# EPOCHDevs/PandasArrow

Measured on AMD Instinct MI355X. Metric: Grows/sec hash group-by-sum, 1e9 int64 rows x 1e6 keys, higher is better.
Workload: dtype f64; 1 GPU; group_by(int64 key).agg(sum,mean,count), 1e+09 rows / 1e+06 keys, 1 GPU; rows=1000000000, keys=1000000, rows_per_gpu=1000000000, parity=bit-exact vs Arrow-order pairwise sum

## Files before the change

### pandasarrow_amd/csrc/compact.hpp

```cpp
#pragma once
#include "pdx_common.hpp"
#include "scan.hpp"

namespace pdx {

constexpr int kCompactBlock = 256;
constexpr int kCompactItems = 16;
constexpr int kCompactTile = kCompactBlock * kCompactItems;

template <typename Pred>
__global__ void __launch_bounds__(kCompactBlock) k_compact_count(int64_t n, Pred pred, int64_t* __restrict__ block_counts) {
  __shared__ int wave_tot[4];
  const int lane = threadIdx.x & 63, wave = threadIdx.x >> 6;
  int64_t base = (int64_t)blockIdx.x * kCompactTile + wave * (64 * kCompactItems);
  int cnt = 0;
  for (int s = 0; s < kCompactItems; ++s) {
    int64_t i = base + s * 64 + lane;
    bool p = i < n && pred(i);
    cnt += __popcll(__ballot(p));
  }
  if (lane == 0) wave_tot[wave] = cnt;
  __syncthreads();
  if (threadIdx.x == 0) block_counts[blockIdx.x] = (int64_t)wave_tot[0] + wave_tot[1] + wave_tot[2] + wave_tot[3];
}
// ... 11 lines not shown
  }
  if (lane == 0) wave_tot[wave] = cnt;
  __syncthreads();
  int64_t pos = block_offsets[blockIdx.x];
  for (int w = 0; w < wave; ++w) pos += wave_tot[w];
  const uint64_t lt = (1ull << lane) - 1ull;
  for (int s = 0; s < kCompactItems; ++s) {
    int64_t i = base + s * 64 + lane;
    bool p = i < n && pred(i);
    uint64_t b = __ballot(p);
    if (p) emit(pos + __popcll(b & lt), i);
    pos += __popcll(b);
  }
}

template <typename Pred, typename Emit>
int compact_indices(int64_t n, Pred pred, Emit emit, int64_t* total_host , Scratch& s,
                    hipStream_t st) {
  if (total_host) *total_host = 0;
  if (n <= 0) return PDX_OK;
  int64_t nblocks = ceil_div(n, kCompactTile);
  int64_t* counts = s.get<int64_t>((size_t)nblocks);
  int64_t* total = s.get<int64_t>(1);
  PDX_SCRATCH_CHECK(s);
  hipLaunchKernelGGL((k_compact_count<Pred>), dim3((unsigned)nblocks), dim3(kCompactBlock), 0, st, n, pred, counts);
  PDX_TRY((device_exclusive_scan<int64_t, SumOp>(counts, counts, nblocks, total, s, st)));
  hipLaunchKernelGGL((k_compact_write<Pred, Emit>), dim3((unsigned)nblocks), dim3(kCompactBlock), 0, st, n, pred, emit, counts);
  PDX_LAUNCH_CHECK();
  if (!total_host) return PDX_OK;
  PDX_HIP(hipMemcpyAsync(total_host, total, sizeof(int64_t), hipMemcpyDeviceToHost, st));
  PDX_HIP(hipStreamSynchronize(st));
  return PDX_OK;
}

template <typename Pred>
int count_if(int64_t n, Pred pred, int64_t* total_host, Scratch& s, hipStream_t st) {
  *total_host = 0;
  if (n <= 0) return PDX_OK;
  int64_t nblocks = ceil_div(n, kCompactTile);
  int64_t* counts = s.get<int64_t>((size_t)nblocks);
  int64_t* total = s.get<int64_t>(1);
  PDX_SCRATCH_CHECK(s);
  hipLaunchKernelGGL((k_compact_count<Pred>), dim3((unsigned)nblocks), dim3(kCompactBlock), 0, st, n, pred, counts);
// ... 21 lines not shown
```

### pandasarrow_amd/csrc/gb_create.hpp

```cpp
#pragma once

struct CreateTuning {
  bool sorted = true;
  bool dense = true;
  bool dense_lds = true;
  bool dense_speculate = true;
  int speculate_bits = 20;
  int64_t prefix_per_slot = 0;
  int partition = 1;
  bool hash_rows = false;
  bool hash_lds = true;
  int64_t head_rows = 0;
  bool hash_split = true;
  bool hash_debug = false;
  static CreateTuning read() {
    CreateTuning t;
    auto off = [](const char* name) { const char* e = getenv(name); return e && e[0] == '0'; };
    t.sorted = !off("PDX_GROUPBY_SORTED");
    t.dense = !off("PDX_GROUPBY_DENSE");
    t.dense_lds = !off("PDX_DENSE_LDS");
    t.dense_speculate = !off("PDX_DENSE_SPECULATE");
    if (const char* e = getenv("PDX_DENSE_SPECULATE_BITS")) t.speculate_bits = atoi(e);
    if (const char* e = getenv("PDX_DENSE_PREFIX_PER_SLOT")) if (atoi(e) > 0) t.prefix_per_slot = atoi(e);
    if (const char* e = getenv("PDX_HASH_PARTITION")) t.partition = e[0] == '0' ? 0 : e[0] == '2' ? 2 : 1;
// ... 12 lines not shown
  const uint8_t* valid;
  int64_t key_off;
  int64_t n;
  Scratch& s;
  hipStream_t st;
  const CreateTuning& t;
  HashCtl* ctl;
};

struct SlotDomain {
  Slot* table = nullptr;
  unsigned int* dense_first = nullptr;
  long long dense_min = 0;
  unsigned int dense_mask = 0, null_slot = 0, region = 0;
  int64_t nslots = 0;
};

struct PoolFree {
  void operator()(void* p) const { pool_free(p); }
};
using TableBlock = std::unique_ptr<Slot, PoolFree>;
static Slot* alloc_table(unsigned int cap) { return static_cast<Slot*>(pool_alloc(((size_t)cap + 2) * sizeof(Slot))); }

constexpr KeyRange kNoKeys{0x7FFFFFFFFFFFFFFFll, (long long)0x8000000000000000ull, 0, 0};
static void widen_range(KeyRange& r, const KeyRange& w) {
  if (!w.any) return;
  r.vmin = std::min(r.vmin, w.vmin);
  r.vmax = std::max(r.vmax, w.vmax);
  r.any = 1;
}

struct KeySample {
  bool maybe_sorted = false;
  KeyRange range = kNoKeys;
};
static int sample_keys(const CreateCtx& c, bool want_sorted, bool want_range, KeySample* out) {
  if (!want_sorted && !want_range) return PDX_OK;
  KeyRange hsv[64];
  unsigned int hflags[4] = {0, 0, 0, 4u};
  unsigned int* flags = c.s.get<unsigned int>(4);
  KeyRange* dsample = c.s.get<KeyRange>(64);
  if (c.s.failed) return PDX_OOM;
  if (want_sorted) {
    PDX_HIP(hipMemsetAsync(flags, 0, 4 * sizeof(unsigned int), c.st));
    hipLaunchKernelGGL(k_sample_descents, dim3(64), dim3(1024), 0, c.st, c.keys, c.valid, c.key_off, c.n, flags + 3);
    PDX_HIP(hipMemcpyAsync(hflags, flags, sizeof(hflags), hipMemcpyDeviceToHost, c.st));
  }
  if (want_range) {
    hipLaunchKernelGGL(k_sample_key_range, dim3(64), dim3(1024), 0, c.st, c.keys, c.valid, c.key_off, c.n, dsample);
    PDX_HIP(hipMemcpyAsync(hsv, dsample, sizeof(hsv), hipMemcpyDeviceToHost, c.st));
  }
  PDX_LAUNCH_CHECK();
  PDX_HIP(hipStreamSynchronize(c.st));
  out->maybe_sorted = want_sorted && !(hflags[3] & 4u) && (hflags[3] & 3u) != 3u;
  if (want_range)
    for (const KeyRange& w : hsv) widen_range(out->range, w);
  return PDX_OK;
}

static int64_t dense_prefix_rows(const CreateCtx& c, int64_t nslots) {
  int64_t per_slot = c.t.prefix_per_slot;
  if (per_slot <= 0) per_slot = c.n < ((int64_t)1 << 29) ? 8 : ((nslots + 31) >> 5) <= kDenseLdsWords ? 4 : 16;
  const int64_t prefix = std::min<int64_t>(c.n, std::max<int64_t>((int64_t)1 << 22, per_slot * nslots));
  return std::min<int64_t>(c.n, round_up(prefix, kSortTile));
}

static int build_dense_domain(const CreateCtx& c, long long mn, unsigned int mask, unsigned int null_slot, int64_t nslots, KeyRange* range_out,
                              unsigned int** first_out) {
  pdx_groupby* gb = c.gb;
  hipStream_t st = c.st;
  const int64_t n = c.n;
  unsigned int* dense_first = *first_out = c.s.get<unsigned int>((size_t)nslots);
  if (c.s.failed) return PDX_OOM;
  hipMemsetAsync(dense_first, 0xFF, (size_t)nslots * sizeof(unsigned int), st);
  const int64_t ntiles = ceil_div(n, kSortTile), nchunks = ceil_div(ntiles, kColChunk);
  const int bits0 = make_sort_plan(ilog2((uint64_t)nslots), sort_max_bits()).bits[0];
  const int64_t prefix = dense_prefix_rows(c, nslots);
  const bool fuse = bits0 >= 4 && bits0 <= 8;
  const int64_t nwords = (nslots + 31) >> 5;
  const int64_t tile_first_tail = prefix / kSortTile;
  const bool lds_bitmap = fuse && c.t.dense_lds && prefix < n && nwords <= kDenseLdsWords && ntiles - tile_first_tail >= 256;
  if (range_out && !(fuse && prefix < n)) return fail(PDX_DEVICE, "dense_build: fused key range needs the histogram tail");
  uint32_t* chunk_sum = nullptr;
  if (fuse) {
    gb->pass0_off = gb->own<uint32_t>((size_t)ntiles << bits0);
    chunk_sum = c.s.get<uint32_t>((size_t)(nchunks + 1) << bits0);
    if (!gb->pass0_off || c.s.failed) return PDX_OOM;
  }
  KeyRange* wg_range = nullptr;
  long long *tile_min = nullptr, *tile_max = nullptr;
  if (range_out) {
    wg_range = c.s.get<KeyRange>((size_t)kCUs);
    if (c.s.failed) return PDX_OOM;
    if (!lds_bitmap) {
      tile_min = c.s.get<long long>((size_t)ntiles);
      tile_max = c.s.get<long long>((size_t)ntiles);
      if (c.s.failed) return PDX_OOM;
    }
  }
  {
    PDX_PROFILE("dense_slots", st);
    if (prefix < n && fuse && (lds_bitmap || range_out))
      hipLaunchKernelGGL(k_dense_slots<false>, dim3(grid_for(prefix, 256, 8)), dim3(256), 0, st, c.keys, c.valid, c.key_off, prefix, mn, mask, null_slot,
                         dense_first, gb->slot_of_row);
    else
      hipLaunchKernelGGL(k_dense_slots<true>, dim3(grid_for(prefix, 256, 8)), dim3(256), 0, st, c.keys, c.valid, c.key_off, prefix, mn, mask, null_slot,
                         dense_first, gb->slot_of_row);
    if (prefix < n) {
// ... 14 lines not shown
                               mask, null_slot, seen, prefix, dense_first, gb->slot_of_row, gb->pass0_off, tile_min, tile_max);
          else
            hipLaunchKernelGGL((k_dense_slots_tail_hist<b()>), dim3(tail_tiles), dim3(kSortBlock), 0, st, c.keys, c.valid, c.key_off, tile_first_tail, n, mn,
                               mask, null_slot, seen, prefix, dense_first, gb->slot_of_row, gb->pass0_off, (long long*)nullptr, (long long*)nullptr);
        });
    }
  }
  PDX_LAUNCH_CHECK();
  if (fuse) {
    if (!lds_bitmap && !range_out)
      with_digit_bits<4, 8>(bits0, [&](auto b) {
        hipLaunchKernelGGL((k_radix_hist<b()>), dim3((unsigned)ceil_div(prefix, kSortTile)), dim3(kSortBlock), 0, st, gb->slot_of_row, prefix, 0, gb->pass0_off);
      });
    PDX_TRY(radix_scan_dispatch(bits0, gb->pass0_off, ntiles, chunk_sum, true, st));
  }
  if (range_out && !lds_bitmap) {
    long long lo = 0, hi = 0, dummy = 0;
    PDX_TRY(minmax_i64_host(tile_min, ntiles, &lo, &dummy, c.s, st));
    PDX_TRY(minmax_i64_host(tile_max, ntiles, &dummy, &hi, c.s, st));
    *range_out = KeyRange{lo, hi, lo <= hi ? 1 : 0, 0};
  } else if (range_out) {
    std::vector<KeyRange> h((size_t)kCUs);
    PDX_HIP(hipMemcpyAsync(h.data(), wg_range, sizeof(KeyRange) * kCUs, hipMemcpyDeviceToHost, st));
    PDX_HIP(hipStreamSynchronize(st));
    *range_out = kNoKeys;
    for (const KeyRange& w : h) widen_range(*range_out, w);
  }
  return PDX_OK;
}

struct KeyRangeFacts {
  MinMaxPartial<long long> mm;
  bool have_mm = false;
  bool not_dense = false;
};

static unsigned long long dense_limit(int64_t n) { return std::min<unsigned long long>(1ull << 26, (unsigned long long)n * 4 + 1024); }

static int try_dense_speculative(const CreateCtx& c, const KeyRange& hs, SlotDomain* d, KeyRangeFacts* f) {
  pdx_groupby* gb = c.gb;
  const int64_t n = c.n;
  const unsigned long long dense_lim = dense_limit(n);
  int b = 64;
  if (hs.any) {
    const unsigned long long span_s = (unsigned long long)hs.vmax - (unsigned long long)hs.vmin;
    b = 4;
    while (b < 64 && (span_s >> b)) ++b;
    if (span_s >= dense_lim) f->not_dense = true;
  }
  if (!(b <= c.t.speculate_bits && b <= 26 && (1ull << b) <= dense_lim && (int64_t)16 * (((int64_t)1 << b) + 1) + 2 * kSortTile < n)) return PDX_OK;
  const unsigned int mask = (1u << b) - 1, null_slot = 1u << b;
  const int64_t nslots = (int64_t)null_slot + (c.valid ? 1 : 0);
  const size_t mark = gb->owned.size();
  gb->slot_of_row = gb->own<uint32_t>((size_t)n);
  if (!gb->slot_of_row) return PDX_OOM;
  KeyRange exact;
  unsigned int* first = nullptr;
  PDX_TRY(build_dense_domain(c, 0, mask, null_slot, nslots, &exact, &first));
  f->mm.vmin = exact.vmin;
  f->mm.vmax = exact.vmax;
  f->mm.rmin = f->mm.rmax = exact.any ? 0 : -1;
  f->have_mm = true;
  if (exact.any && (unsigned long long)exact.vmax - (unsigned long long)exact.vmin <= mask) {
    gb->dense = 1;
    d->dense_first = first;
    d->dense_min = exact.vmin;
    d->dense_mask = mask;
    d->null_slot = null_slot;
    d->nslots = nslots;
    return PDX_OK;
  }
  while (gb->owned.size() > mark) {
    pool_free(gb->owned.back());
    gb->owned.pop_back();
  }
  gb->slot_of_row = nullptr;
  gb->pass0_off = nullptr;
  return PDX_OK;
}

static int try_dense_exact(const CreateCtx& c, SlotDomain* d, KeyRangeFacts* f) {
  pdx_groupby* gb = c.gb;
  if (!f->have_mm) {
    PDX_TRY(minmax_keys_host(c.keys, c.valid, c.key_off, c.n, &f->mm, c.s, c.st));
    f->have_mm = true;
  }
  if (f->mm.rmin >= 0) {
    const unsigned long long span = (unsigned long long)f->mm.vmax - (unsigned long long)f->mm.vmin;
    if (span >= dense_limit(c.n)) return PDX_OK;
    d->dense_min = f->mm.vmin;
    d->null_slot = (unsigned int)span + 1;
    d->nslots = (int64_t)d->null_slot + 1;
  } else {
    d->null_slot = 0;
    d->nslots = 1;
  }
  gb->dense = 1;
  gb->slot_of_row = gb->own<uint32_t>((size_t)c.n);
  if (!gb->slot_of_row) return PDX_OOM;
  return build_dense_domain(c, d->dense_min, 0, d->null_slot, d->nslots, nullptr, &d->dense_first);
}

struct HashPartition {
  int64_t ntiles = 0, nchunks = 0;
  long long* keys_part = nullptr;
  unsigned int pb = kPartBits;
  uint32_t* bucket_starts = nullptr;
  bool idx16_written = false;
  bool lds_failed_at_pb = false;
};

static int partition_by_bucket(const CreateCtx& c, HashPartition* hp) {
  pdx_groupby* gb = c.gb;
  hipStream_t st = c.st;
  const int64_t n = c.n;
// ... 220 lines not shown
  gb->owned.push_back(table.get());
  d->table = table.release();
  d->null_slot = cap;
  d->nslots = (int64_t)cap + 2;
  return PDX_OK;
}

static int finish_group_ids(const CreateCtx& c, const SlotDomain& d) {
  pdx_groupby* gb = c.gb;
  Scratch& s = c.s;
  hipStream_t st = c.st;
  const int64_t n = c.n, nslots = d.nslots;
  gb->nslots = nslots;
  gb->slot_bits = ilog2((uint64_t)nslots);
  gb->gid_of_slot = gb->own<uint32_t>((size_t)nslots);
  uint32_t* occ_slot_tmp = s.get<uint32_t>((size_t)std::min<int64_t>(nslots, n + 2));
  uint32_t* occ_first_tmp = s.get<uint32_t>((size_t)std::min<int64_t>(nslots, n + 2));
  if (s.failed || !gb->gid_of_slot) return PDX_OOM;
  int64_t G = 0;
  PDX_TRY(compact_indices(nslots, OccPred{d.table, d.dense_first, d.region, d.null_slot},
                          OccEmit{d.table, d.dense_first, d.region, d.null_slot, occ_slot_tmp, occ_first_tmp}, &G, s, st));
  gb->G = G;
  gb->occ_slot = gb->own<uint32_t>((size_t)G);
  gb->gid_of_occ = gb->own<uint32_t>((size_t)G);
  gb->uniques = gb->own<int64_t>((size_t)G);
  gb->unique_ok = gb->own<uint8_t>((size_t)G);
  gb->first_rows = gb->own<int64_t>((size_t)G);
  if (s.failed || !gb->occ_slot || !gb->gid_of_occ || !gb->uniques || !gb->unique_ok || !gb->first_rows) return PDX_OOM;
  hipMemcpyAsync(gb->occ_slot, occ_slot_tmp, (size_t)G * sizeof(uint32_t), hipMemcpyDeviceToDevice, st);
  const bool rank_by_sort = G > ((int64_t)1 << 22) && G * 8 > n;
  const int g = grid_for(G, 256);
  if (rank_by_sort) {
    uint32_t* k0 = s.get<uint32_t>((size_t)G);
    uint32_t* v0 = s.get<uint32_t>((size_t)G);
    uint32_t* k1 = s.get<uint32_t>((size_t)G);
    uint32_t* v1 = s.get<uint32_t>((size_t)G);
    PDX_SCRATCH_CHECK(s);
    const uint32_t *ks = nullptr, *vs = nullptr;
    PDX_TRY(radix_sort_pairs<uint32_t>(occ_first_tmp, occ_slot_tmp, k0, v0, k1, v1, G, ilog2((uint64_t)n + 1) < 31 ? ilog2((uint64_t)n + 1) : 31, &ks, &vs, true,
                                       s, st));
    hipLaunchKernelGGL(k_assign_gids, dim3(g), dim3(256), 0, st, d.table, d.dense_min, d.dense_mask, gb->gid_of_slot, ks, vs, G, d.null_slot, gb->uniques,
                       gb->unique_ok, gb->first_rows, d.region);
    hipLaunchKernelGGL(k_gid_of_occ, dim3(g), dim3(256), 0, st, gb->gid_of_slot, gb->occ_slot, G, gb->gid_of_occ);
  } else {
    const int64_t nwords = (n + 63) >> 6, nrb = ceil_div(nwords, (int64_t)kRankWords);
    unsigned long long* bits = s.get<unsigned long long>((size_t)nwords);
    int64_t* block_pre = s.get<int64_t>((size_t)nrb);
    PDX_SCRATCH_CHECK(s);
    PDX_HIP(hipMemsetAsync(bits, 0, (size_t)nwords * sizeof(unsigned long long), st));
    hipLaunchKernelGGL(k_mark_first_rows, dim3(g), dim3(256), 0, st, occ_first_tmp, G, bits);
    hipLaunchKernelGGL(k_rank_block_counts, dim3(grid_for(nrb * kRankWords, 256)), dim3(256), 0, st, bits, nwords, nrb, block_pre);
    PDX_TRY((device_exclusive_scan<int64_t, SumOp>(block_pre, block_pre, nrb, (int64_t*)nullptr, s, st)));
    hipLaunchKernelGGL(k_assign_gids_ranked, dim3(g), dim3(256), 0, st, d.table, d.dense_min, d.dense_mask, gb->gid_of_slot, occ_first_tmp, occ_slot_tmp, G, bits,
                       block_pre, d.null_slot, gb->uniques, gb->unique_ok, gb->first_rows, d.region, gb->gid_of_occ);
  }
  return PDX_OK;
}
```

### pandasarrow_amd/csrc/gb_dense_slots.hpp

```cpp
#pragma once

__device__ __forceinline__ unsigned int dense_slot_of(long long k, long long mn, unsigned int mask) {
  return mask ? ((unsigned int)(unsigned long long)k & mask) : (unsigned int)((unsigned long long)k - (unsigned long long)mn);
}
struct KeyRange {
  long long vmin, vmax;
  int any, pad;
};
__global__ void __launch_bounds__(1024) k_sample_key_range(const long long* __restrict__ keys, const uint8_t* __restrict__ valid, int64_t off,
                                                           int64_t n, KeyRange* __restrict__ out) {
  __shared__ long long smn[16], smx[16];
  __shared__ int sany[16];
  const int64_t nsamp = n < 65536 ? n : 65536;
  long long mn = 0x7FFFFFFFFFFFFFFFll, mx = (long long)0x8000000000000000ull;
  int any = 0;
  {
    const int64_t j = (int64_t)blockIdx.x * 1024 + threadIdx.x;
    int64_t i = j < nsamp ? (int64_t)((unsigned __int128)j * (unsigned __int128)n / (unsigned __int128)nsamp) : n;
    if (i < n && (!valid || bit_get(valid, off + i))) {
      long long k = keys[i];
      mn = k < mn ? k : mn;
      mx = k > mx ? k : mx;
      any = 1;
    }
  }
  for (int d = 32; d >= 1; d >>= 1) {
    long long a = __shfl_xor(mn, d, 64), b = __shfl_xor(mx, d, 64);
    int c = __shfl_xor(any, d, 64);
    mn = a < mn ? a : mn;
    mx = b > mx ? b : mx;
    any |= c;
  }
  if ((threadIdx.x & 63) == 0) {
    smn[threadIdx.x >> 6] = mn;
    smx[threadIdx.x >> 6] = mx;
    sany[threadIdx.x >> 6] = any;
  }
  __syncthreads();
  if (threadIdx.x == 0) {
    for (int w = 1; w < 16; ++w) {
      mn = smn[w] < mn ? smn[w] : mn;
      mx = smx[w] > mx ? smx[w] : mx;
      any |= sany[w];
    }
    out[blockIdx.x].vmin = mn;
    out[blockIdx.x].vmax = mx;
    out[blockIdx.x].any = any;
  }
}
template <bool WRITE_SLOTS>
__global__ void __launch_bounds__(256) k_dense_slots(const long long* __restrict__ keys, const uint8_t* __restrict__ valid, int64_t off,
                                                     int64_t n, long long mn, unsigned int mask, unsigned int range, unsigned int* first,
                                                     uint32_t* __restrict__ slot_of_row) {
  int64_t stride = (int64_t)gridDim.x * blockDim.x;
  for (int64_t i = (int64_t)blockIdx.x * blockDim.x + threadIdx.x; i < n; i += stride) {
    unsigned int s = range;
    if (!valid || bit_get(valid, off + i)) s = dense_slot_of(ld_stream<kStreamDenseKeys>(keys + i), mn, mask);
    if constexpr (WRITE_SLOTS) st_stream<kStreamDenseSlots>(slot_of_row + i, s);
    const bool want = (unsigned int)i < first[s];
    const int lane = threadIdx.x & 63;
    uint64_t rem = __ballot(want);
    for (int rounds = 0; rem && rounds < 4; ++rounds) {
// ... 130 lines not shown
constexpr int kDenseLdsWords = 32768;
constexpr int kDenseLdsBlock = 1024;
template <int BITS>
__global__ void __launch_bounds__(kDenseLdsBlock) k_dense_slots_tail_hist_lds(const long long* __restrict__ keys, const uint8_t* __restrict__ valid,
                                                                              int64_t off, int64_t tile0, int64_t ntiles, int64_t n, long long mn,
                                                                              unsigned int mask, unsigned int range,
                                                                              const uint32_t* __restrict__ seen, int nwords, int64_t track_from,
                                                                              unsigned int* first, uint32_t* __restrict__ slot_of_row,
                                                                              uint32_t* __restrict__ hist, KeyRange* __restrict__ range_out) {
  constexpr int R = 1 << BITS;
  constexpr int W = kDenseLdsBlock / 64;
  __shared__ uint32_t lseen[kDenseLdsWords];
  __shared__ uint32_t lh[W][R];
  __shared__ long long smn[W], smx[W];
  __shared__ int sany[W];
  for (int i = threadIdx.x; i < nwords; i += kDenseLdsBlock) lseen[i] = seen[i];
  for (int i = threadIdx.x; i < W * R; i += kDenseLdsBlock) (&lh[0][0])[i] = 0;
  __syncthreads();
  const int lane = threadIdx.x & 63, wave = threadIdx.x >> 6;
  const int64_t nw = (int64_t)gridDim.x * W;
  long long kmn = 0x7FFFFFFFFFFFFFFFll, kmx = (long long)0x8000000000000000ull;
  int any = 0;
  bool few = true;
  auto count_and_track = [&](bool in, unsigned int sl, int64_t i) {
    const uint32_t w = lseen[sl >> 5];
    const unsigned int d = sl & (R - 1);
    if (few) {
      uint64_t rem = __ballot(in);
      int rounds = 0;
      while (rem && rounds < 4) {
        const int leader = __ffsll((unsigned long long)rem) - 1;
        const unsigned int dl = (unsigned int)__shfl((int)d, leader, 64);
        const uint64_t grp = __ballot(in && d == dl) & rem;
        if (lane == leader) atomicAdd(&lh[wave][dl], (uint32_t)__popcll(grp));
        rem &= ~grp;
        ++rounds;
      }
      if (rem) {
        few = false;
        if ((rem >> lane) & 1) atomicAdd(&lh[wave][d], 1u);
      }
    } else if (in) {
      atomicAdd(&lh[wave][d], 1u);
    }
    if (in && !((w >> (sl & 31)) & 1u) && i >= track_from) {
      if ((unsigned int)i < first[sl]) atomicMin(&first[sl], (unsigned int)i);
    }
  };
  const bool can_wide = PDX_DENSE_WIDE && !valid && ((reinterpret_cast<uintptr_t>(keys) | reinterpret_cast<uintptr_t>(slot_of_row)) & 15) == 0;
  for (int64_t tile = tile0 + (int64_t)blockIdx.x * W + wave; tile < ntiles; tile += nw) {
    const int64_t base = tile * kSortTile;
    if (can_wide && base + kSortTile <= n) {
#pragma unroll 1
      for (int c = 0; c < kSortTile / 1024; ++c) {
        const i64x2* kp = reinterpret_cast<const i64x2*>(keys + base + c * 1024) + 2 * lane;
        u32x4* sp = reinterpret_cast<u32x4*>(slot_of_row + base + c * 1024) + lane;
        i64x2 k2[8];
#pragma unroll
        for (int u = 0; u < 4; ++u) {
          k2[2 * u] = ld_stream<kStreamDenseKeys>(kp + u * 128);
          k2[2 * u + 1] = ld_stream<kStreamDenseKeys>(kp + u * 128 + 1);
// ... 36 lines not shown
          }
          if (in) st_stream<kStreamDenseSlots>(slot_of_row + i, sl);
          count_and_track(in, sl, i);
        }
      }
    }
    for (int d = lane; d < R; d += 64) {
      hist[tile * R + d] = lh[wave][d];
      lh[wave][d] = 0;
    }
  }
  if (range_out) {
    for (int d = 32; d >= 1; d >>= 1) {
      long long a = __shfl_xor(kmn, d, 64), b = __shfl_xor(kmx, d, 64);
      int c = __shfl_xor(any, d, 64);
      kmn = a < kmn ? a : kmn;
      kmx = b > kmx ? b : kmx;
      any |= c;
    }
    if (lane == 0) {
      smn[wave] = kmn;
      smx[wave] = kmx;
      sany[wave] = any;
    }
    __syncthreads();
    if (threadIdx.x == 0) {
      for (int w = 1; w < W; ++w) {
        kmn = smn[w] < kmn ? smn[w] : kmn;
        kmx = smx[w] > kmx ? smx[w] : kmx;
        any |= sany[w];
      }
      range_out[blockIdx.x].vmin = kmn;
      range_out[blockIdx.x].vmax = kmx;
      range_out[blockIdx.x].any = any;
    }
  }
}
```

### pandasarrow_amd/csrc/gb_resample_kernels.hpp

```cpp
#pragma once

struct BinParams {
  const long long* ts;
  long long first, freq;
  double inv_freq;
  int closed_right;
  __device__ long long bin(int64_t i) const {
    long long x = ts[i] - first - (closed_right ? 1 : 0);
    long long q = (long long)((double)x * inv_freq);
    long long r = x - q * freq;
    while (r < 0) { --q; r += freq; }
    while (r >= freq) { ++q; r -= freq; }
    return q;
  }
};
__global__ void k_bin_lower_bounds(BinParams p, int64_t n, int64_t nbins, long long tmin, long long tmax, uint32_t* __restrict__ lb ) {
  int64_t stride = (int64_t)gridDim.x * blockDim.x;
  const double scale = tmax > tmin ? (double)(n - 1) / (double)(tmax - tmin) : 0.0;
  for (int64_t b = (int64_t)blockIdx.x * blockDim.x + threadIdx.x; b <= nbins; b += stride) {
    if (b == nbins) {
      lb[b] = (uint32_t)n;
      continue;
    }
    long long edge = p.first + b * p.freq;
// ... 78 lines not shown
  int64_t stride = (int64_t)gridDim.x * blockDim.x;
  for (int64_t i = (int64_t)blockIdx.x * blockDim.x + threadIdx.x; i < n; i += stride) {
    int64_t lo = 0, hi = G;
    while (hi - lo > 1) {
      int64_t mid = (lo + hi) >> 1;
      if (seg_start[mid] <= (uint32_t)i) lo = mid;
      else hi = mid;
    }
    out[i] = (uint32_t)lo;
  }
}
__global__ void k_set_last(uint32_t* p, int64_t idx, uint32_t v) {
  if (threadIdx.x == 0 && blockIdx.x == 0) p[idx] = v;
}

__global__ void __launch_bounds__(1024) k_sample_descents(const long long* __restrict__ keys, const uint8_t* __restrict__ valid, int64_t off, int64_t n,
                                                          unsigned int* __restrict__ flags) {
  const int64_t npairs = n - 1;
  const int64_t nsamp = npairs < 65536 ? npairs : 65536;
  const int64_t j = (int64_t)blockIdx.x * 1024 + threadIdx.x;
  if (j >= nsamp) return;
  const int64_t i = (int64_t)((unsigned __int128)j * (unsigned __int128)npairs / (unsigned __int128)nsamp);
  unsigned int f = 0;
  if (valid && (!bit_get(valid, off + i) || !bit_get(valid, off + i + 1))) f |= 4u;
  const long long a = keys[i], b = keys[i + 1];
  if (b < a) f |= 1u;
  if ((unsigned long long)b < (unsigned long long)a) f |= 2u;
  if (f) atomicOr(flags, f);
}
constexpr int kRunBlock = 256, kRunSteps = 16, kRunTile = kRunBlock * kRunSteps;
constexpr int kRunWaveRows = 64 * kRunSteps;
template <typename LabelFn, int BATCH>
__global__ void __launch_bounds__(kRunBlock) k_label_run_count(int64_t n, LabelFn fn, unsigned long long* __restrict__ marks,
                                                                int64_t* __restrict__ wave_counts, unsigned int* __restrict__ flags) {
  static_assert(kRunSteps % BATCH == 0, "whole batches");
  const int lane = threadIdx.x & 63;
  const int64_t w = ((int64_t)blockIdx.x * kRunBlock + threadIdx.x) >> 6;
  const int64_t base = w * kRunWaveRows;
  if (base >= n) return;
  long long last = 0;
  if (lane == 0 && base > 0) last = fn(base - 1);
  int cnt = 0;
  bool desc_s = false, desc_u = false;
  auto step = [&](int s, long long label) {
// ... 75 lines not shown
```

### pandasarrow_amd/csrc/radix_sort.hpp

```cpp
#pragma once
#include <stdlib.h>
#include <type_traits>
#include "pdx_common.hpp"
#include "scan.hpp"
#include "stream_io.hpp"

namespace pdx {

constexpr int kSortBlock = 256;
constexpr int kSortItems = 16;
constexpr int kSortTile = kSortBlock * kSortItems;
constexpr int kSortWaves = kSortBlock / 64;
constexpr uint32_t kSortKeyMask = 0x7FFFFFFFu;
constexpr int kScatBlock = 256;
constexpr int kScatItems = kSortTile / kScatBlock;
constexpr int kScatWaves = kScatBlock / 64;

__device__ __forceinline__ void wave_hist_add(uint32_t* h, uint32_t d, uint32_t& cand) {
  const unsigned long long m = __ballot(d == cand);
  const int shared = __popcll(m);
  if (shared >= 8) {
    if (d != cand) atomicAdd(&h[d], 1u);
    else if ((int)__lane_id() == __ffsll((long long)m) - 1) atomicAdd(&h[d], (uint32_t)shared);
  } else {
// ... 36 lines not shown
        }
      }
    }
  } else {
#pragma unroll
    for (int k = 0; k < kSortItems; ++k) {
      int64_t i = base + k * kSortBlock + threadIdx.x;
      if (i < n) wave_hist_add(h, ((uint32_t)ld_stream<kStreamHistKeys>(keys + i) >> shift) & (R - 1), cand);
    }
  }
  __syncthreads();
  for (int d = threadIdx.x; d < R; d += kSortBlock) hist[(int64_t)blockIdx.x * R + d] = h[d];
}

constexpr int kColChunk = 256;
template <int BITS>
__global__ void __launch_bounds__(256) k_col_chunk_sums(const uint32_t* __restrict__ hist, int64_t ntiles,
                                                        uint32_t* __restrict__ chunk_sum ) {
  constexpr int R = 1 << BITS;
  constexpr int T = R >= 256 ? 1 : 256 / R;
  int64_t t0 = (int64_t)blockIdx.x * kColChunk;
  int64_t t1 = t0 + kColChunk < ntiles ? t0 + kColChunk : ntiles;
  if constexpr (T == 1) {
    for (int d = threadIdx.x; d < R; d += 256) {
      uint32_t acc = 0;
      for (int64_t t = t0; t < t1; ++t) acc += hist[t * R + d];
      chunk_sum[(int64_t)blockIdx.x * R + d] = acc;
    }
  } else {
    __shared__ uint32_t part[256];
    const int tl = threadIdx.x / R, d = threadIdx.x % R;
    uint32_t acc = 0;
    for (int64_t t = t0 + tl; t < t1; t += T) acc += hist[t * R + d];
    part[threadIdx.x] = acc;
    __syncthreads();
    if (tl == 0) {
#pragma unroll
// ... 35 lines not shown
      tsum += t[j];
    }
    uint32_t total;
    uint32_t pre = block_exclusive_scan(tsum, SumOp(), &total, smem);
#pragma unroll
    for (int j = 0; j < DPT; ++j) {
      int d = threadIdx.x * DPT + j;
      if (d < R) dpre[d] = pre;
      pre += t[j];
    }
    __syncthreads();
  }
  int64_t t0 = (int64_t)blockIdx.x * kColChunk;
  int64_t t1 = t0 + kColChunk < ntiles ? t0 + kColChunk : ntiles;
  constexpr int T = R >= 256 ? 1 : 256 / R;
  if constexpr (T == 1) {
    for (int d = threadIdx.x; d < R; d += 256) {
      uint32_t off = chunk_off[(int64_t)blockIdx.x * R + d] + dpre[d];
      for (int64_t t = t0; t < t1; ++t) {
        uint32_t v = hist[t * R + d];
        hist[t * R + d] = off;
        off += v;
      }
    }
  } else {
    __shared__ uint32_t part[256];
    const int tl = threadIdx.x / R, d = threadIdx.x % R;
    const int64_t sub = (t1 - t0 + T - 1) / T;
    const int64_t ts = t0 + tl * sub, te = ts + sub < t1 ? ts + sub : t1;
    uint32_t acc = 0;
// ... 518 lines not shown
```

Before: 69.69 Grows/s.

## Merge key sampling kernels, precount occupancy early, bound rank bitmap, vectorize column scans

Merges the sorted-check and key-range sampling kernels into one launch with a single host copy. In the dense LDS path, the occupied-slot count is enqueued before the existing range readback, so one sync serves both, and the later compaction only writes straight into the final occ_slot buffer with no device-to-device copy. The dense kernel also records the highest first-occurrence row, which bounds the first-row bitmap used in ranking. The radix column chunk-sum and offset kernels gain u32x4 vectorized paths for radices between 16 and 1024. Together these aim to cut launches, host syncs and memory traffic, at the cost of more code paths and alignment-dependent branches.

```diff
diff --git a/pandasarrow_amd/csrc/compact.hpp b/pandasarrow_amd/csrc/compact.hpp
--- a/pandasarrow_amd/csrc/compact.hpp
+++ b/pandasarrow_amd/csrc/compact.hpp
@@ -49,19 +49,33 @@
   }
 }
 
+template <typename Pred>
+int compact_count_enqueue(int64_t n, Pred pred, int64_t** offsets_out, int64_t* total, Scratch& s, hipStream_t st) {
+  int64_t nblocks = ceil_div(n, kCompactTile);
+  int64_t* counts = *offsets_out = s.get<int64_t>((size_t)nblocks);
+  PDX_SCRATCH_CHECK(s);
+  hipLaunchKernelGGL((k_compact_count<Pred>), dim3((unsigned)nblocks), dim3(kCompactBlock), 0, st, n, pred, counts);
+  PDX_TRY((device_exclusive_scan<int64_t, SumOp>(counts, counts, nblocks, total, s, st)));
+  PDX_LAUNCH_CHECK();
+  return PDX_OK;
+}
+template <typename Pred, typename Emit>
+int compact_write_enqueue(int64_t n, Pred pred, Emit emit, const int64_t* offsets, hipStream_t st) {
+  hipLaunchKernelGGL((k_compact_write<Pred, Emit>), dim3((unsigned)ceil_div(n, kCompactTile)), dim3(kCompactBlock), 0, st, n, pred, emit, offsets);
+  PDX_LAUNCH_CHECK();
+  return PDX_OK;
+}
+
 template <typename Pred, typename Emit>
 int compact_indices(int64_t n, Pred pred, Emit emit, int64_t* total_host , Scratch& s,
                     hipStream_t st) {
   if (total_host) *total_host = 0;
   if (n <= 0) return PDX_OK;
-  int64_t nblocks = ceil_div(n, kCompactTile);
-  int64_t* counts = s.get<int64_t>((size_t)nblocks);
+  int64_t* counts = nullptr;
   int64_t* total = s.get<int64_t>(1);
   PDX_SCRATCH_CHECK(s);
-  hipLaunchKernelGGL((k_compact_count<Pred>), dim3((unsigned)nblocks), dim3(kCompactBlock), 0, st, n, pred, counts);
-  PDX_TRY((device_exclusive_scan<int64_t, SumOp>(counts, counts, nblocks, total, s, st)));
-  hipLaunchKernelGGL((k_compact_write<Pred, Emit>), dim3((unsigned)nblocks), dim3(kCompactBlock), 0, st, n, pred, emit, counts);
-  PDX_LAUNCH_CHECK();
+  PDX_TRY(compact_count_enqueue(n, pred, &counts, total, s, st));
+  PDX_TRY(compact_write_enqueue(n, pred, emit, counts, st));
   if (!total_host) return PDX_OK;
   PDX_HIP(hipMemcpyAsync(total_host, total, sizeof(int64_t), hipMemcpyDeviceToHost, st));
   PDX_HIP(hipStreamSynchronize(st));
diff --git a/pandasarrow_amd/csrc/gb_create.hpp b/pandasarrow_amd/csrc/gb_create.hpp
--- a/pandasarrow_amd/csrc/gb_create.hpp
+++ b/pandasarrow_amd/csrc/gb_create.hpp
@@ -50,6 +50,9 @@
   long long dense_min = 0;
   unsigned int dense_mask = 0, null_slot = 0, region = 0;
   int64_t nslots = 0;
+  int64_t first_row_bound = 0;
+  int64_t* occ_offsets = nullptr;
+  int64_t occupied = 0;
 };
 
 struct PoolFree {
@@ -72,25 +75,19 @@
 };
 static int sample_keys(const CreateCtx& c, bool want_sorted, bool want_range, KeySample* out) {
   if (!want_sorted && !want_range) return PDX_OK;
-  KeyRange hsv[64];
-  unsigned int hflags[4] = {0, 0, 0, 4u};
-  unsigned int* flags = c.s.get<unsigned int>(4);
-  KeyRange* dsample = c.s.get<KeyRange>(64);
+  KeySampleWg h[64];
+  KeySampleWg* dsample = c.s.get<KeySampleWg>(64);
   if (c.s.failed) return PDX_OOM;
-  if (want_sorted) {
-    PDX_HIP(hipMemsetAsync(flags, 0, 4 * sizeof(unsigned int), c.st));
-    hipLaunchKernelGGL(k_sample_descents, dim3(64), dim3(1024), 0, c.st, c.keys, c.valid, c.key_off, c.n, flags + 3);
-    PDX_HIP(hipMemcpyAsync(hflags, flags, sizeof(hflags), hipMemcpyDeviceToHost, c.st));
-  }
-  if (want_range) {
-    hipLaunchKernelGGL(k_sample_key_range, dim3(64), dim3(1024), 0, c.st, c.keys, c.valid, c.key_off, c.n, dsample);
-    PDX_HIP(hipMemcpyAsync(hsv, dsample, sizeof(hsv), hipMemcpyDeviceToHost, c.st));
-  }
+  hipLaunchKernelGGL(k_sample_keys, dim3(64), dim3(1024), 0, c.st, c.keys, c.valid, c.key_off, c.n, (int)want_sorted, (int)want_range, dsample);
   PDX_LAUNCH_CHECK();
+  PDX_HIP(hipMemcpyAsync(h, dsample, sizeof(h), hipMemcpyDeviceToHost, c.st));
   PDX_HIP(hipStreamSynchronize(c.st));
-  out->maybe_sorted = want_sorted && !(hflags[3] & 4u) && (hflags[3] & 3u) != 3u;
-  if (want_range)
-    for (const KeyRange& w : hsv) widen_range(out->range, w);
+  unsigned int descents = 0;
+  for (const KeySampleWg& w : h) {
+    descents |= w.descents;
+    if (want_range) widen_range(out->range, KeyRange{w.vmin, w.vmax, w.any, 0});
+  }
+  out->maybe_sorted = want_sorted && !(descents & 4u) && (descents & 3u) != 3u;
   return PDX_OK;
 }
 
@@ -102,11 +99,11 @@
 }
 
 static int build_dense_domain(const CreateCtx& c, long long mn, unsigned int mask, unsigned int null_slot, int64_t nslots, KeyRange* range_out,
-                              unsigned int** first_out) {
-  pdx_groupby* gb = c.gb;
-  hipStream_t st = c.st;
-  const int64_t n = c.n;
-  unsigned int* dense_first = *first_out = c.s.get<unsigned int>((size_t)nslots);
+                              SlotDomain* d) {
+  pdx_groupby* gb = c.gb;
+  hipStream_t st = c.st;
+  const int64_t n = c.n;
+  unsigned int* dense_first = d->dense_first = c.s.get<unsigned int>((size_t)nslots);
   if (c.s.failed) return PDX_OOM;
   hipMemsetAsync(dense_first, 0xFF, (size_t)nslots * sizeof(unsigned int), st);
   const int64_t ntiles = ceil_div(n, kSortTile), nchunks = ceil_div(ntiles, kColChunk);
@@ -125,9 +122,11 @@
   }
   KeyRange* wg_range = nullptr;
   long long *tile_min = nullptr, *tile_max = nullptr;
+  if (lds_bitmap) {
+    wg_range = c.s.get<KeyRange>((size_t)kCUs + 1);
+    if (c.s.failed) return PDX_OOM;
+  }
   if (range_out) {
-    wg_range = c.s.get<KeyRange>((size_t)kCUs);
-    if (c.s.failed) return PDX_OOM;
     if (!lds_bitmap) {
       tile_min = c.s.get<long long>((size_t)ntiles);
       tile_max = c.s.get<long long>((size_t)ntiles);
@@ -172,17 +171,27 @@
       });
     PDX_TRY(radix_scan_dispatch(bits0, gb->pass0_off, ntiles, chunk_sum, true, st));
   }
-  if (range_out && !lds_bitmap) {
+  if (lds_bitmap) {
+    static_assert(sizeof(KeyRange) % sizeof(int64_t) == 0, "the count sits behind the KeyRange array");
+    int64_t* occupied = reinterpret_cast<int64_t*>(wg_range + kCUs);
+    PDX_TRY(compact_count_enqueue(nslots, OccPred{nullptr, dense_first, 0, null_slot}, &d->occ_offsets, occupied, c.s, st));
+    std::vector<KeyRange> h((size_t)kCUs + 1);
+    PDX_HIP(hipMemcpyAsync(h.data(), wg_range, sizeof(KeyRange) * (kCUs + 1), hipMemcpyDeviceToHost, st));
+    PDX_HIP(hipStreamSynchronize(st));
+    KeyRange exact = kNoKeys;
+    unsigned int track_end = 0;
+    for (int w = 0; w < kCUs; ++w) {
+      widen_range(exact, h[(size_t)w]);
+      track_end = std::max(track_end, h[(size_t)w].track_end);
+    }
+    if (range_out) *range_out = exact;
+    memcpy(&d->occupied, &h[(size_t)kCUs], sizeof(int64_t));
+    d->first_row_bound = std::max<int64_t>(prefix, (int64_t)track_end);
+  } else if (range_out) {
     long long lo = 0, hi = 0, dummy = 0;
     PDX_TRY(minmax_i64_host(tile_min, ntiles, &lo, &dummy, c.s, st));
     PDX_TRY(minmax_i64_host(tile_max, ntiles, &dummy, &hi, c.s, st));
     *range_out = KeyRange{lo, hi, lo <= hi ? 1 : 0, 0};
-  } else if (range_out) {
-    std::vector<KeyRange> h((size_t)kCUs);
-    PDX_HIP(hipMemcpyAsync(h.data(), wg_range, sizeof(KeyRange) * kCUs, hipMemcpyDeviceToHost, st));
-    PDX_HIP(hipStreamSynchronize(st));
-    *range_out = kNoKeys;
-    for (const KeyRange& w : h) widen_range(*range_out, w);
   }
   return PDX_OK;
 }
@@ -213,15 +222,13 @@
   gb->slot_of_row = gb->own<uint32_t>((size_t)n);
   if (!gb->slot_of_row) return PDX_OOM;
   KeyRange exact;
-  unsigned int* first = nullptr;
-  PDX_TRY(build_dense_domain(c, 0, mask, null_slot, nslots, &exact, &first));
+  PDX_TRY(build_dense_domain(c, 0, mask, null_slot, nslots, &exact, d));
   f->mm.vmin = exact.vmin;
   f->mm.vmax = exact.vmax;
   f->mm.rmin = f->mm.rmax = exact.any ? 0 : -1;
   f->have_mm = true;
   if (exact.any && (unsigned long long)exact.vmax - (unsigned long long)exact.vmin <= mask) {
     gb->dense = 1;
-    d->dense_first = first;
     d->dense_min = exact.vmin;
     d->dense_mask = mask;
     d->null_slot = null_slot;
@@ -234,6 +241,7 @@
   }
   gb->slot_of_row = nullptr;
   gb->pass0_off = nullptr;
+  *d = SlotDomain{};
   return PDX_OK;
 }
 
@@ -256,7 +264,7 @@
   gb->dense = 1;
   gb->slot_of_row = gb->own<uint32_t>((size_t)c.n);
   if (!gb->slot_of_row) return PDX_OOM;
-  return build_dense_domain(c, d->dense_min, 0, d->null_slot, d->nslots, nullptr, &d->dense_first);
+  return build_dense_domain(c, d->dense_min, 0, d->null_slot, d->nslots, nullptr, d);
 }
 
 struct HashPartition {
@@ -507,20 +515,32 @@
   gb->nslots = nslots;
   gb->slot_bits = ilog2((uint64_t)nslots);
   gb->gid_of_slot = gb->own<uint32_t>((size_t)nslots);
-  uint32_t* occ_slot_tmp = s.get<uint32_t>((size_t)std::min<int64_t>(nslots, n + 2));
-  uint32_t* occ_first_tmp = s.get<uint32_t>((size_t)std::min<int64_t>(nslots, n + 2));
+  const int64_t max_occ = std::min<int64_t>(nslots, n + 2);
+  uint32_t* occ_first_tmp = s.get<uint32_t>((size_t)max_occ);
   if (s.failed || !gb->gid_of_slot) return PDX_OOM;
   int64_t G = 0;
-  PDX_TRY(compact_indices(nslots, OccPred{d.table, d.dense_first, d.region, d.null_slot},
-                          OccEmit{d.table, d.dense_first, d.region, d.null_slot, occ_slot_tmp, occ_first_tmp}, &G, s, st));
+  const OccPred occupied{d.table, d.dense_first, d.region, d.null_slot};
+  const uint32_t* occ_slots = nullptr;
+  if (d.occ_offsets) {
+    G = d.occupied;
+    occ_slots = gb->occ_slot = gb->own<uint32_t>((size_t)G);
+    if (!gb->occ_slot) return PDX_OOM;
+    PDX_TRY(compact_write_enqueue(nslots, occupied, OccEmit{d.table, d.dense_first, d.region, d.null_slot, gb->occ_slot, occ_first_tmp}, d.occ_offsets, st));
+  } else {
+    uint32_t* occ_slot_tmp = s.get<uint32_t>((size_t)max_occ);
+    PDX_SCRATCH_CHECK(s);
+    PDX_TRY(compact_indices(nslots, occupied, OccEmit{d.table, d.dense_first, d.region, d.null_slot, occ_slot_tmp, occ_first_tmp}, &G, s, st));
+    gb->occ_slot = gb->own<uint32_t>((size_t)G);
+    if (!gb->occ_slot) return PDX_OOM;
+    PDX_HIP(hipMemcpyAsync(gb->occ_slot, occ_slot_tmp, (size_t)G * sizeof(uint32_t), hipMemcpyDeviceToDevice, st));
+    occ_slots = occ_slot_tmp;
+  }
   gb->G = G;
-  gb->occ_slot = gb->own<uint32_t>((size_t)G);
   gb->gid_of_occ = gb->own<uint32_t>((size_t)G);
   gb->uniques = gb->own<int64_t>((size_t)G);
   gb->unique_ok = gb->own<uint8_t>((size_t)G);
   gb->first_rows = gb->own<int64_t>((size_t)G);
-  if (s.failed || !gb->occ_slot || !gb->gid_of_occ || !gb->uniques || !gb->unique_ok || !gb->first_rows) return PDX_OOM;
-  hipMemcpyAsync(gb->occ_slot, occ_slot_tmp, (size_t)G * sizeof(uint32_t), hipMemcpyDeviceToDevice, st);
+  if (s.failed || !gb->gid_of_occ || !gb->uniques || !gb->unique_ok || !gb->first_rows) return PDX_OOM;
   const bool rank_by_sort = G > ((int64_t)1 << 22) && G * 8 > n;
   const int g = grid_for(G, 256);
   if (rank_by_sort) {
@@ -530,13 +550,14 @@
     uint32_t* v1 = s.get<uint32_t>((size_t)G);
     PDX_SCRATCH_CHECK(s);
     const uint32_t *ks = nullptr, *vs = nullptr;
-    PDX_TRY(radix_sort_pairs<uint32_t>(occ_first_tmp, occ_slot_tmp, k0, v0, k1, v1, G, ilog2((uint64_t)n + 1) < 31 ? ilog2((uint64_t)n + 1) : 31, &ks, &vs, true,
+    PDX_TRY(radix_sort_pairs<uint32_t>(occ_first_tmp, occ_slots, k0, v0, k1, v1, G, ilog2((uint64_t)n + 1) < 31 ? ilog2((uint64_t)n + 1) : 31, &ks, &vs, true,
                                        s, st));
     hipLaunchKernelGGL(k_assign_gids, dim3(g), dim3(256), 0, st, d.table, d.dense_min, d.dense_mask, gb->gid_of_slot, ks, vs, G, d.null_slot, gb->uniques,
                        gb->unique_ok, gb->first_rows, d.region);
     hipLaunchKernelGGL(k_gid_of_occ, dim3(g), dim3(256), 0, st, gb->gid_of_slot, gb->occ_slot, G, gb->gid_of_occ);
   } else {
-    const int64_t nwords = (n + 63) >> 6, nrb = ceil_div(nwords, (int64_t)kRankWords);
+    const int64_t bound = d.first_row_bound > 0 ? std::min(d.first_row_bound, n) : n;
+    const int64_t nwords = (bound + 63) >> 6, nrb = ceil_div(nwords, (int64_t)kRankWords);
     unsigned long long* bits = s.get<unsigned long long>((size_t)nwords);
     int64_t* block_pre = s.get<int64_t>((size_t)nrb);
     PDX_SCRATCH_CHECK(s);
@@ -544,7 +565,7 @@
     hipLaunchKernelGGL(k_mark_first_rows, dim3(g), dim3(256), 0, st, occ_first_tmp, G, bits);
     hipLaunchKernelGGL(k_rank_block_counts, dim3(grid_for(nrb * kRankWords, 256)), dim3(256), 0, st, bits, nwords, nrb, block_pre);
     PDX_TRY((device_exclusive_scan<int64_t, SumOp>(block_pre, block_pre, nrb, (int64_t*)nullptr, s, st)));
-    hipLaunchKernelGGL(k_assign_gids_ranked, dim3(g), dim3(256), 0, st, d.table, d.dense_min, d.dense_mask, gb->gid_of_slot, occ_first_tmp, occ_slot_tmp, G, bits,
+    hipLaunchKernelGGL(k_assign_gids_ranked, dim3(g), dim3(256), 0, st, d.table, d.dense_min, d.dense_mask, gb->gid_of_slot, occ_first_tmp, occ_slots, G, bits,
                        block_pre, d.null_slot, gb->uniques, gb->unique_ok, gb->first_rows, d.region, gb->gid_of_occ);
   }
   return PDX_OK;
diff --git a/pandasarrow_amd/csrc/gb_dense_slots.hpp b/pandasarrow_amd/csrc/gb_dense_slots.hpp
--- a/pandasarrow_amd/csrc/gb_dense_slots.hpp
+++ b/pandasarrow_amd/csrc/gb_dense_slots.hpp
@@ -5,23 +5,40 @@
 }
 struct KeyRange {
   long long vmin, vmax;
-  int any, pad;
+  int any;
+  unsigned int track_end;
 };
-__global__ void __launch_bounds__(1024) k_sample_key_range(const long long* __restrict__ keys, const uint8_t* __restrict__ valid, int64_t off,
-                                                           int64_t n, KeyRange* __restrict__ out) {
+struct KeySampleWg {
+  long long vmin, vmax;
+  int any;
+  unsigned int descents;
+};
+__global__ void __launch_bounds__(1024) k_sample_keys(const long long* __restrict__ keys, const uint8_t* __restrict__ valid, int64_t off, int64_t n,
+                                                      int want_descents, int want_range, KeySampleWg* __restrict__ out) {
   __shared__ long long smn[16], smx[16];
   __shared__ int sany[16];
-  const int64_t nsamp = n < 65536 ? n : 65536;
+  __shared__ unsigned int sdesc[16];
   long long mn = 0x7FFFFFFFFFFFFFFFll, mx = (long long)0x8000000000000000ull;
   int any = 0;
-  {
-    const int64_t j = (int64_t)blockIdx.x * 1024 + threadIdx.x;
+  unsigned int f = 0;
+  const int64_t j = (int64_t)blockIdx.x * 1024 + threadIdx.x;
+  if (want_range) {
+    const int64_t nsamp = n < 65536 ? n : 65536;
     int64_t i = j < nsamp ? (int64_t)((unsigned __int128)j * (unsigned __int128)n / (unsigned __int128)nsamp) : n;
     if (i < n && (!valid || bit_get(valid, off + i))) {
-      long long k = keys[i];
-      mn = k < mn ? k : mn;
-      mx = k > mx ? k : mx;
+      mn = mx = keys[i];
       any = 1;
+    }
+  }
+  if (want_descents) {
+    const int64_t npairs = n - 1;
+    const int64_t nsamp = npairs < 65536 ? npairs : 65536;
+    if (j < nsamp) {
+      const int64_t i = (int64_t)((unsigned __int128)j * (unsigned __int128)npairs / (unsigned __int128)nsamp);
+      if (valid && (!bit_get(valid, off + i) || !bit_get(valid, off + i + 1))) f |= 4u;
+      const long long a = keys[i], b = keys[i + 1];
+      if (b < a) f |= 1u;
+      if ((unsigned long long)b < (unsigned long long)a) f |= 2u;
     }
   }
   for (int d = 32; d >= 1; d >>= 1) {
@@ -30,11 +47,13 @@
     mn = a < mn ? a : mn;
     mx = b > mx ? b : mx;
     any |= c;
+    f |= (unsigned int)__shfl_xor((int)f, d, 64);
   }
   if ((threadIdx.x & 63) == 0) {
     smn[threadIdx.x >> 6] = mn;
     smx[threadIdx.x >> 6] = mx;
     sany[threadIdx.x >> 6] = any;
+    sdesc[threadIdx.x >> 6] = f;
   }
   __syncthreads();
   if (threadIdx.x == 0) {
@@ -42,10 +61,12 @@
       mn = smn[w] < mn ? smn[w] : mn;
       mx = smx[w] > mx ? smx[w] : mx;
       any |= sany[w];
+      f |= sdesc[w];
     }
     out[blockIdx.x].vmin = mn;
     out[blockIdx.x].vmax = mx;
     out[blockIdx.x].any = any;
+    out[blockIdx.x].descents = f;
   }
 }
 template <bool WRITE_SLOTS>
@@ -206,6 +227,7 @@
   __shared__ uint32_t lh[W][R];
   __shared__ long long smn[W], smx[W];
   __shared__ int sany[W];
+  __shared__ unsigned int send[W];
   for (int i = threadIdx.x; i < nwords; i += kDenseLdsBlock) lseen[i] = seen[i];
   for (int i = threadIdx.x; i < W * R; i += kDenseLdsBlock) (&lh[0][0])[i] = 0;
   __syncthreads();
@@ -213,6 +235,7 @@
   const int64_t nw = (int64_t)gridDim.x * W;
   long long kmn = 0x7FFFFFFFFFFFFFFFll, kmx = (long long)0x8000000000000000ull;
   int any = 0;
+  unsigned int track_end = 0;
   bool few = true;
   auto count_and_track = [&](bool in, unsigned int sl, int64_t i) {
     const uint32_t w = lseen[sl >> 5];
@@ -236,7 +259,10 @@
       atomicAdd(&lh[wave][d], 1u);
     }
     if (in && !((w >> (sl & 31)) & 1u) && i >= track_from) {
-      if ((unsigned int)i < first[sl]) atomicMin(&first[sl], (unsigned int)i);
+      if ((unsigned int)i < first[sl]) {
+        atomicMin(&first[sl], (unsigned int)i);
+        track_end = (unsigned int)i + 1u > track_end ? (unsigned int)i + 1u : track_end;
+      }
     }
   };
   const bool can_wide = PDX_DENSE_WIDE && !valid && ((reinterpret_cast<uintptr_t>(keys) | reinterpret_cast<uintptr_t>(slot_of_row)) & 15) == 0;
@@ -303,14 +329,17 @@
     for (int d = 32; d >= 1; d >>= 1) {
       long long a = __shfl_xor(kmn, d, 64), b = __shfl_xor(kmx, d, 64);
       int c = __shfl_xor(any, d, 64);
+      const unsigned int e = (unsigned int)__shfl_xor((int)track_end, d, 64);
       kmn = a < kmn ? a : kmn;
       kmx = b > kmx ? b : kmx;
       any |= c;
+      track_end = e > track_end ? e : track_end;
     }
     if (lane == 0) {
       smn[wave] = kmn;
       smx[wave] = kmx;
       sany[wave] = any;
+      send[wave] = track_end;
     }
     __syncthreads();
     if (threadIdx.x == 0) {
@@ -318,10 +347,12 @@
         kmn = smn[w] < kmn ? smn[w] : kmn;
         kmx = smx[w] > kmx ? smx[w] : kmx;
         any |= sany[w];
+        track_end = send[w] > track_end ? send[w] : track_end;
       }
       range_out[blockIdx.x].vmin = kmn;
       range_out[blockIdx.x].vmax = kmx;
       range_out[blockIdx.x].any = any;
-    }
-  }
-}
+      range_out[blockIdx.x].track_end = track_end;
+    }
+  }
+}
diff --git a/pandasarrow_amd/csrc/gb_resample_kernels.hpp b/pandasarrow_amd/csrc/gb_resample_kernels.hpp
--- a/pandasarrow_amd/csrc/gb_resample_kernels.hpp
+++ b/pandasarrow_amd/csrc/gb_resample_kernels.hpp
@@ -116,20 +116,6 @@
   if (threadIdx.x == 0 && blockIdx.x == 0) p[idx] = v;
 }
 
-__global__ void __launch_bounds__(1024) k_sample_descents(const long long* __restrict__ keys, const uint8_t* __restrict__ valid, int64_t off, int64_t n,
-                                                          unsigned int* __restrict__ flags) {
-  const int64_t npairs = n - 1;
-  const int64_t nsamp = npairs < 65536 ? npairs : 65536;
-  const int64_t j = (int64_t)blockIdx.x * 1024 + threadIdx.x;
-  if (j >= nsamp) return;
-  const int64_t i = (int64_t)((unsigned __int128)j * (unsigned __int128)npairs / (unsigned __int128)nsamp);
-  unsigned int f = 0;
-  if (valid && (!bit_get(valid, off + i) || !bit_get(valid, off + i + 1))) f |= 4u;
-  const long long a = keys[i], b = keys[i + 1];
-  if (b < a) f |= 1u;
-  if ((unsigned long long)b < (unsigned long long)a) f |= 2u;
-  if (f) atomicOr(flags, f);
-}
 constexpr int kRunBlock = 256, kRunSteps = 16, kRunTile = kRunBlock * kRunSteps;
 constexpr int kRunWaveRows = 64 * kRunSteps;
 template <typename LabelFn, int BATCH>
diff --git a/pandasarrow_amd/csrc/radix_sort.hpp b/pandasarrow_amd/csrc/radix_sort.hpp
--- a/pandasarrow_amd/csrc/radix_sort.hpp
+++ b/pandasarrow_amd/csrc/radix_sort.hpp
@@ -74,6 +74,11 @@
 }
 
 constexpr int kColChunk = 256;
+template <int R>
+constexpr bool kColWide = R >= 16 && R <= 1024;
+__device__ __forceinline__ bool col_tables_aligned(const void* a, const void* b) {
+  return ((reinterpret_cast<uintptr_t>(a) | reinterpret_cast<uintptr_t>(b)) & 15) == 0;
+}
 template <int BITS>
 __global__ void __launch_bounds__(256) k_col_chunk_sums(const uint32_t* __restrict__ hist, int64_t ntiles,
                                                         uint32_t* __restrict__ chunk_sum ) {
@@ -81,6 +86,31 @@
   constexpr int T = R >= 256 ? 1 : 256 / R;
   int64_t t0 = (int64_t)blockIdx.x * kColChunk;
   int64_t t1 = t0 + kColChunk < ntiles ? t0 + kColChunk : ntiles;
+  if constexpr (kColWide<R>) {
+    if (col_tables_aligned(hist, chunk_sum)) {
+      constexpr int V = R / 4, TW = 256 / V;
+      __shared__ u32x4 part4[256];
+      const int tl = threadIdx.x / V, q = threadIdx.x % V;
+      const u32x4* col = reinterpret_cast<const u32x4*>(hist) + q;
+      u32x4 acc = {0u, 0u, 0u, 0u};
+      int64_t t = t0 + tl;
+      for (; t + 7 * TW < t1; t += 8 * TW) {
+        u32x4 v[8];
+#pragma unroll
+        for (int u = 0; u < 8; ++u) v[u] = col[(t + u * TW) * V];
+#pragma unroll
+        for (int u = 0; u < 8; ++u) acc += v[u];
+      }
+      for (; t < t1; t += TW) acc += col[t * V];
+      part4[threadIdx.x] = acc;
+      __syncthreads();
+      if (tl == 0) {
+        for (int j = 1; j < TW; ++j) acc += part4[j * V + q];
+        reinterpret_cast<u32x4*>(chunk_sum)[(int64_t)blockIdx.x * V + q] = acc;
+      }
+      return;
+    }
+  }
   if constexpr (T == 1) {
     for (int d = threadIdx.x; d < R; d += 256) {
       uint32_t acc = 0;
@@ -146,6 +176,69 @@
   int64_t t0 = (int64_t)blockIdx.x * kColChunk;
   int64_t t1 = t0 + kColChunk < ntiles ? t0 + kColChunk : ntiles;
   constexpr int T = R >= 256 ? 1 : 256 / R;
+  if constexpr (kColWide<R>) {
+    if (col_tables_aligned(hist, chunk_off)) {
+      constexpr int V = R / 4, TW = 256 / V;
+      constexpr int NT = kColChunk / TW;
+      constexpr bool kKeep = NT <= 32;
+      __shared__ u32x4 part4[256];
+      const int tl = threadIdx.x / V, q = threadIdx.x % V;
+      u32x4* col = reinterpret_cast<u32x4*>(hist) + q;
+      const int64_t ts = t0 + (int64_t)tl * NT;
+      const int cnt = ts < t1 ? (int)(t1 - ts < NT ? t1 - ts : NT) : 0;
+      u32x4 acc = {0u, 0u, 0u, 0u};
+      u32x4 keep[kKeep ? NT : 1];
+      if constexpr (kKeep) {
+#pragma unroll
+        for (int u = 0; u < NT; ++u) keep[u] = col[(ts + u < t1 ? ts + u : t1 - 1) * V];
+#pragma unroll
+        for (int u = 0; u < NT; ++u) {
+          if (u >= cnt) keep[u] = u32x4{0u, 0u, 0u, 0u};
+          acc += keep[u];
+        }
+      } else {
+        int u0 = 0;
+        for (; u0 + 8 <= cnt; u0 += 8) {
+          u32x4 v[8];
+#pragma unroll
+          for (int u = 0; u < 8; ++u) v[u] = col[(ts + u0 + u) * V];
+#pragma unroll
+          for (int u = 0; u < 8; ++u) acc += v[u];
+        }
+        for (; u0 < cnt; ++u0) acc += col[(ts + u0) * V];
+      }
+      part4[threadIdx.x] = acc;
+      __syncthreads();
+      u32x4 off = reinterpret_cast<const u32x4*>(chunk_off)[(int64_t)blockIdx.x * V + q];
+      off += u32x4{dpre[4 * q], dpre[4 * q + 1], dpre[4 * q + 2], dpre[4 * q + 3]};
+      for (int j = 0; j < tl; ++j) off += part4[j * V + q];
+      if constexpr (kKeep) {
+#pragma unroll
+        for (int u = 0; u < NT; ++u) {
+          if (u < cnt) col[(ts + u) * V] = off;
+          off += keep[u];
+        }
+      } else {
+        int u0 = 0;
+        for (; u0 + 8 <= cnt; u0 += 8) {
+          u32x4 v[8];
+#pragma unroll
+          for (int u = 0; u < 8; ++u) v[u] = col[(ts + u0 + u) * V];
+#pragma unroll
+          for (int u = 0; u < 8; ++u) {
+            col[(ts + u0 + u) * V] = off;
+            off += v[u];
+          }
+        }
+        for (; u0 < cnt; ++u0) {
+          const u32x4 v = col[(ts + u0) * V];
+          col[(ts + u0) * V] = off;
+          off += v;
+        }
+      }
+      return;
+    }
+  }
   if constexpr (T == 1) {
     for (int d = threadIdx.x; d < R; d += 256) {
       uint32_t off = chunk_off[(int64_t)blockIdx.x * R + d] + dpre[d];
```

After: 69.54 Grows/s. No clear change (-0.2%).
